# sd196821/QuadSim

Hardware: AMD Instinct MI355X
Metric: env-steps/sec at N parallel envs (1/2/4/8 GPU); per-step state L2 err vs NumPy ref (higher is better)
Workload: dtype f32

## Files before the change

quadsim_amd/csrc/kernel_diag.hpp:

```cpp
#pragma once

#ifdef QS_STAMP
#define QS_STAMP_DECL unsigned long long stamp_[8] = {0, 0, 0, 0, 0, 0, 0, 0}; (void)stamp_
#if QS_STAMP + 0 >= 2
#define QS_STAMP_AT(slot)                                                                                       \
    do {                                                                                                        \
         \
         \
         \
         \
        if ((slot) == 1) stamp_[0] = __builtin_amdgcn_s_memrealtime();                                          \
        else if ((slot) == (role == 0 ? 7 : 6)) {                                                               \
            if (lane == 0 && A.stamps && (tile & 63) == 0) {                    \
                const unsigned long long now_ = __builtin_amdgcn_s_memrealtime();                               \
                const unsigned long long ix_ = ((k0 % 64ull) * (unsigned long long)(A.stamp_tiles) + (unsigned long long)tile) * 16ull + 8 * role; \
                if (ix_ + 8 <= A.stamp_cap) { A.stamps[ix_] = stamp_[0]; A.stamps[ix_ + (slot)] = now_; }       \
            }                                                                                                   \
        }                                                                                                       \
    } while (0)
#else
#define QS_STAMP_AT(slot) (stamp_[slot] = __builtin_amdgcn_s_memrealtime())
#endif
#if QS_STAMP + 0 >= 2
#define QS_STAMP_FLUSH() ((void)0)
#else
#define QS_STAMP_FLUSH()                                                                                        \
    do {                                                                                                        \
        if (lane == 0 && A.stamps) {                                                                            \
            const unsigned long long ix_ = ((k0 % 64ull) * (unsigned long long)(A.stamp_tiles) + (unsigned long long)tile) * 16ull + 8 * role; \
            if (ix_ + 8 <= A.stamp_cap) for (int j_ = 0; j_ < 8; ++j_) A.stamps[ix_ + j_] = stamp_[j_];          \
        }                                                                                                       \
    } while (0)
#endif
#define QS_PHASE_DECL unsigned long long ph_[8] = {0, 0, 0, 0, 0, 0, 0, 0}, ph_t_ = __builtin_amdgcn_s_memrealtime(); \
    const unsigned long long ph_c0_ = __builtin_amdgcn_s_memtime(), ph_r0_ = ph_t_
#define QS_PHASE(slot) do { const unsigned long long n_ = __builtin_amdgcn_s_memrealtime(); ph_[slot] += n_ - ph_t_; ph_t_ = n_; } while (0)
#define QS_PHASE_FLUSH(role_)                                                                                   \
    do {                                                                                                        \
        ph_[6] = __builtin_amdgcn_s_memtime() - ph_c0_;                                   \
        ph_[7] = __builtin_amdgcn_s_memrealtime() - ph_r0_;       \
        if (lane == 0 && A.stamps) {                                                                            \
            const unsigned long long ix_ = (unsigned long long)tile * 16ull + 8 * (role_);                      \
            if (ix_ + 8 <= A.stamp_cap) for (int j_ = 0; j_ < 8; ++j_) A.stamps[ix_ + j_] = ph_[j_];             \
        }                                                                                                       \
    } while (0)
#else
#define QS_STAMP_DECL ((void)0)
#define QS_STAMP_AT(slot) ((void)0)
#define QS_STAMP_FLUSH() ((void)0)
#define QS_PHASE_DECL ((void)0)
#define QS_PHASE(slot) ((void)0)
#define QS_PHASE_FLUSH(role_) ((void)0)
#endif

#if defined(QS_PLAIN_STORES)
#define QS_ST(p, v) (*(p) = (v))
#define QS_SO(p, v) QS_ST(p, v)
#else
#define QS_ST(p, v) __builtin_nontemporal_store((v), (p))
#define QS_SO(p, v) QS_ST(p, v)
#endif
```

quadsim_amd/csrc/private_queue.hpp:

```cpp
#pragma once

struct QsChainLane {
    hsa_queue_t *queue = nullptr;
    char *kernargs = nullptr;
    std::vector<uint64_t> slot_qidx;
    uint64_t issued = 0;
    int64_t tile0 = 0, tile_end = 0;
    hsa_signal_t done{};
    void *rev_ptr = nullptr;
    hsa_signal_t rev{};
    int64_t rev_value = 0;
    char *res_kernarg = nullptr;
    hsa_signal_t res_done{};
    bool res_launched = false;
    uint64_t res_prog = 0;
};

struct QsKernel {
    uint64_t object = 0;
    uint32_t kernarg_size = 0, group_size = 0, private_size = 0;
    unsigned block = 0;
};

struct QsChain {
// ... 375 lines not shown
        memset((char *)p + 4, 0, 60);
        p->signal = wait_sig;
        p->value = wait_value;
        p->mask = -1;
        p->cond = HSA_SIGNAL_CONDITION_GTE;
        p->completion_signal = completion;
        word0 = (uint16_t)((HSA_PACKET_TYPE_VENDOR_SPECIFIC << HSA_PACKET_HEADER_TYPE) | fences) |
                ((uint32_t)HSA_AMD_PACKET_TYPE_BARRIER_VALUE << 16);
    } else {
        hsa_kernel_dispatch_packet_t *p = (hsa_kernel_dispatch_packet_t *)slot;
        const bool res = kind == PKT_RESIDENT;
        p->workgroup_size_x = (uint16_t)(res ? c->res_kernel.block : c->block); p->workgroup_size_y = 1; p->workgroup_size_z = 1;
        p->reserved0 = 0;
        p->grid_size_x = grid; p->grid_size_y = 1; p->grid_size_z = 1;
        p->private_segment_size = res ? c->res_kernel.private_size : c->private_size;
        p->group_segment_size = res ? c->res_kernel.group_size : c->group_size;
        p->kernel_object = res ? c->res_kernel.object : c->kernel_object;
        p->kernarg_address = (void *)kernarg;
        p->reserved2 = 0;
        p->completion_signal = completion;
        word0 = (uint16_t)((HSA_PACKET_TYPE_KERNEL_DISPATCH << HSA_PACKET_HEADER_TYPE) | fences) |
                ((uint32_t)(1 << HSA_KERNEL_DISPATCH_PACKET_SETUP_DIMENSIONS) << 16);
    }
    __atomic_store_n((uint32_t *)slot, word0, __ATOMIC_RELEASE);
    hsa_signal_store_screlease(L.queue->doorbell_signal, (hsa_signal_value_t)idx);
    return idx;
}


double res_now()
{
    timespec ts;
    clock_gettime(CLOCK_MONOTONIC, &ts);
    return (double)ts.tv_sec + 1e-9 * (double)ts.tv_nsec;
}

int res_resolve_kernel(QsEnv *e)
{
    QsChain *c = e->chain;
    if (!c->v_split) { c->res_fits = false; return QS_OK; }
    if (c->res_kernel.object && c->v_integ == c->rv_integ && c->v_params == c->rv_params && c->v_rmode == c->rv_rmode && c->v_prep == c->rv_prep)
        return QS_OK;
    char sym[200];
    snprintf(sym, sizeof sym, "_ZN12_GLOBAL__N_114k_env_residentILi%dELb%dELi%dELi%dEEEvNS_8StepArgsENS_7ResArgsE.kd", c->v_integ,
             c->v_params, c->v_rmode, c->v_prep);
    hsa_executable_symbol_t ks;
    QsKernel k;
    HSA_TRY(hsa_executable_get_symbol_by_name(c->exe, sym, &c->gpu, &ks));
    HSA_TRY(hsa_executable_symbol_get_info(ks, HSA_EXECUTABLE_SYMBOL_INFO_KERNEL_OBJECT, &k.object));
    HSA_TRY(hsa_executable_symbol_get_info(ks, HSA_EXECUTABLE_SYMBOL_INFO_KERNEL_KERNARG_SEGMENT_SIZE, &k.kernarg_size));
    HSA_TRY(hsa_executable_symbol_get_info(ks, HSA_EXECUTABLE_SYMBOL_INFO_KERNEL_GROUP_SEGMENT_SIZE, &k.group_size));
    HSA_TRY(hsa_executable_symbol_get_info(ks, HSA_EXECUTABLE_SYMBOL_INFO_KERNEL_PRIVATE_SEGMENT_SIZE, &k.private_size));
    if (k.kernarg_size > kResKernargBytes) return fail(QS_ERR_HIP, "queue mode: kernel argument block of %s is %u B", sym, k.kernarg_size);
    const int waves = split_waves(c->v_rmode, c->v_prep);
    k.block = (unsigned)(waves * kTile);
    c->res_kernel = k;
    c->rv_integ = c->v_integ; c->rv_params = c->v_params; c->rv_rmode = c->v_rmode; c->rv_prep = c->v_prep;
    c->res_fits = k.private_size == 0 && e->tiles * waves <= c->res_wave_cap;
    return QS_OK;
}

bool res_running(const QsChainLane &L) { return L.res_launched && hsa_signal_load_relaxed(L.res_done) != 0; }

int res_launch(QsEnv *e, QsChainLane &L, uint64_t seq0, uint64_t stop_seq)
{
    QsChain *c = e->chain;
    const size_t q = (size_t)(&L - c->lanes.data());
    StepArgs A = make_args(e);
    A.tile0 = L.tile0; A.tile_end = L.tile_end;
    A.T = 1;
    ResArgs R{};
    R.ring = c->ring;
    R.rseq = c->d_rseq;
    R.wcnt = c->d_rcnt + q * 32;
    R.fin = R.wcnt + kResWinSlots;
    R.h_prog = c->d_hres + q * 8;
    R.h_fin = R.h_prog + 1;
    R.seq0 = seq0;
    R.base = c->res_seq0;
    R.stop_seq = stop_seq;
    R.slots_mask = c->ring_slots - 1;
    R.idle_ticks = c->res_idle_ticks;
    R.lane_tiles = (unsigned)(L.tile_end - L.tile0);
    const size_t roff = (sizeof(StepArgs) + alignof(ResArgs) - 1) / alignof(ResArgs) * alignof(ResArgs);
    memcpy(L.res_kernarg, &A, sizeof A);
    memcpy(L.res_kernarg + roff, &R, sizeof R);
    __builtin_ia32_sfence();
    (void)*(volatile uint32_t *)(L.res_kernarg + roff + sizeof R - sizeof(uint32_t));
    hsa_signal_store_relaxed(L.res_done, 1);
    chain_write_packet(c, L, PKT_RESIDENT, L.res_kernarg, (unsigned)((L.tile_end - L.tile0) * c->res_kernel.block),
                       HSA_FENCE_SCOPE_SYSTEM, HSA_FENCE_SCOPE_SYSTEM, L.res_done);
    L.res_launched = true;
    ++c->res_dispatches;
    return QS_OK;
}

void res_refresh(QsChain *c)
{
    uint64_t m = UINT64_MAX;
    for (size_t q = 0; q < c->lanes.size(); ++q) {
        QsChainLane &L = c->lanes[q];
        L.res_prog = std::max<uint64_t>(L.res_prog, c->h_res[q * 8]);
        m = std::min<uint64_t>(m, L.res_prog);
    }
    c->res_retired = std::max<uint64_t>(c->res_retired, m);
}

int res_write(QsEnv *e, uint64_t s, int cmd, const StepArgs *A)
{
    QsChain *c = e->chain;
    if (c->res_retired + c->ring_slots <= s) {
        const double t_end = res_now() + kResTimeoutS;
        for (;;) {
            res_refresh(c);
            if (c->res_retired + c->ring_slots > s) break;
            for (QsChainLane &L : c->lanes)
                if (L.res_launched && !res_running(L)) { int r = res_launch(e, L, 0, UINT64_MAX); if (r) return r; }
            if (res_now() > t_end)
                return fail(QS_ERR_HIP, "queue mode: the resident step kernel consumed no descriptor for %.0f s (descriptor %llu, all "
                            "consumed below %llu, first lane's progress %llu, %llu dispatches)", kResTimeoutS, (unsigned long long)s,
                            (unsigned long long)c->res_retired, (unsigned long long)c->h_res[0], (unsigned long long)c->res_dispatches);
            __builtin_ia32_pause();
        }
    }
    const unsigned long long p[7] = {
        A ? (unsigned long long)A->actions : 0, A ? (unsigned long long)A->obs : 0, A ? (unsigned long long)A->reward : 0,
        A ? (unsigned long long)A->done : 0, A ? (unsigned long long)A->flags : 0, A ? (unsigned long long)A->term_obs : 0,
        A ? (unsigned long long)A->term_state : 0};
    for (int i = 0; i < 7; ++i)
        if (p[i] & ~kResPtrMask) return fail(QS_ERR_INVALID, "queue mode: a buffer address above 2^48");
    const unsigned long long tag = (unsigned long long)(s & 0xffff) << 48;
    volatile unsigned long long *w = c->ring + (s & (c->ring_slots - 1)) * kResWords;
    for (int i = 0; i < 7; ++i) w[i] = p[i] | tag;
    w[7] = ((unsigned long long)cmd << 32) | (unsigned long long)(uint32_t)(s >> 16) | tag;
    __builtin_ia32_sfence();
    return QS_OK;
}

int res_finish(QsEnv *e)
{
    QsChain *c = e->chain;
    if (!c->res_open) return QS_OK;
    const uint64_t s = c->res_issued;
    int r = res_write(e, s, 1, nullptr);
    if (r) return r;
    c->res_issued = s + 1;
    const double t_end = res_now() + kResTimeoutS;
    for (;;) {
        bool all = true;
        for (size_t q = 0; q < c->lanes.size(); ++q) {
            QsChainLane &L = c->lanes[q];
            if (res_running(L)) { all = false; continue; }
            if (hsa_signal_load_scacquire(L.res_done) == 0 && c->h_res[q * 8 + 1] >= s + 1) continue;
            r = res_launch(e, L, 0, s + 1);
            if (r) return r;
            all = false;
        }
        if (all) break;
        if (res_now() > t_end)
            return fail(QS_ERR_HIP, "queue mode: the resident step kernel did not end within %.0f s of its EXIT descriptor", kResTimeoutS);
        __builtin_ia32_pause();
    }
    c->res_retired = s + 1;
    c->res_open = false;
    return QS_OK;
}
// ... 160 lines not shown
```

quadsim_amd/csrc/quadsim_hip.hip:

```cpp
#include <hip/hip_runtime.h>
#include <hsa/hsa.h>
#include <hsa/hsa_ext_amd.h>
#include <hsa/amd_hsa_signal.h>

#include <elf.h>
#include <fcntl.h>
#include <sys/mman.h>
#include <sys/stat.h>
#include <unistd.h>

#include <cstdarg>
#include <cstdio>
#include <cstdlib>
#include <cstring>
#include <dlfcn.h>
#include <algorithm>
#include <atomic>
#include <condition_variable>
#include <mutex>
#include <new>
#include <thread>
#include <vector>

#ifdef QS_DEBUG
#include <cassert>
#define QS_ASSERT(c) assert(c)
#else
#define QS_ASSERT(c) ((void)0)
#endif

#include "../../include/quadsim.h"
#include "host_util.hpp"
#include "quadsim_device.hpp"
#include "rollout_ops.hpp"
#include "mlp.hpp"

using namespace qs;

#include "kernel_diag.hpp"
#include "step_kernels.hpp"
#include "layer1_kernels.hpp"
#include "policy_kernels.hpp"
#include "runner_kernels.hpp"
#include "expert_rollout.hpp"
#include "shooting.hpp"

#ifdef QS_STAMP
static unsigned long long *g_host_stamps = nullptr;
static unsigned long long g_host_stamp_cap = 0;
#endif

struct QsEnv {
    QsConfig cfg;
    int64_t n = 0, tiles = 0;
    float *st = nullptr, *par = nullptr;
    bool per_env_params = false;
    hipStream_t stream = nullptr;
    bool own_stream = false;
    unsigned long long *d_ctr = nullptr;
    hipEvent_t ev0 = nullptr, ev1 = nullptr;
    float nominal_obs[12] = {0};
    float *gae_ws = nullptr;
    size_t gae_ws_floats = 0;
    float *init = nullptr;
    int obs_dim = 12;
    HostStage stage;
    std::vector<struct QsGroup *> groups;
    hipEvent_t fork_ev = nullptr;
    bool main_dirty = true;
    bool groups_dirty = false;
    bool runner_env_major = false;
    struct QsChain *chain = nullptr;
};

namespace {

StepArgs make_args(const QsEnv *e)
{
    StepArgs A;
    memset(&A, 0, sizeof A);
    A.st = e->st;
    A.par = e->par;
    A.n = e->n;
    A.tile0 = 0; A.tile_end = e->tiles;
    A.io_env0 = 0; A.io_n = e->n;
    A.T = 1;
    A.step_idx = 0;
    A.ctr = e->d_ctr;
    A.gid0 = e->cfg.env_id_offset;
    A.C.kind = e->cfg.kind == QS_KIND_DOCKING_V2 ? 1 : 0;
    A.C.dt = e->cfg.dt;
    A.C.rmax = e->cfg.kind == QS_KIND_DOCKING_V2 ? 10.0f : 3.0f;
    A.C.vdes_x = e->cfg.kind == QS_KIND_DOCKING_V2 ? 0.2f : 0.0f;
    A.init = e->init;
    A.rc.seed = e->cfg.seed;
    for (int i = 0; i < 4; ++i) A.rc.rr[i] = e->cfg.init_range[i];
    A.rc.rr[4] = e->cfg.mass_scale[0]; A.rc.rr[5] = e->cfg.mass_scale[1];
    A.rc.rr[6] = e->cfg.inertia_scale[0]; A.rc.rr[7] = e->cfg.inertia_scale[1];
    A.rc.par_nom[0] = e->cfg.mass;
    for (int i = 0; i < 3; ++i) A.rc.par_nom[1 + i] = e->cfg.inertia[i];
    A.par_nom = Par{e->cfg.mass, e->cfg.inertia[0], e->cfg.inertia[1], e->cfg.inertia[2]};
    A.auto_reset = e->cfg.auto_reset;
    A.randomise = e->cfg.randomise;

    for (int i = 0; i < 12; ++i) A.nominal_obs[i] = e->nominal_obs[i];
#ifdef QS_STAMP
    A.stamps = g_host_stamps; A.stamp_cap = g_host_stamp_cap; A.stamp_tiles = (unsigned long long)e->tiles;
#endif
    return A;
}

UserIO user_io(QsEnv *e) { return UserIO(e->cfg.io_space == QS_IO_HOST ? &e->stage : nullptr, e->stream); }

std::atomic<int> &prep_forced()
{
    static std::atomic<int> f{getenv("QS_RESET_PREP") ? atoi(getenv("QS_RESET_PREP")) : -1};
    return f;
}

int prep_for(int rmode, int64_t tiles)
{
    const int forced = prep_forced().load(std::memory_order_relaxed);
    if (rmode != 1 && rmode != 2) return 0;
    if (forced == 0 || forced == 2) return forced;
    return tiles <= kPrepMaxTiles ? 2 : 0;
}

enum StepFamily { kFamSerial = 0, kFamSplit = 1, kFamResident = 2, kFamChainSplit = 3, kFamChainSerial = 4, kFamHover = 5 };
struct StepVariant {
    int family, integ, params, rmode, prep;
};

// ... 60 lines not shown
    template __global__ void k_env_resident<I, true, 1, 2>(StepArgs, ResArgs);                                          \
    template __global__ void k_env_resident<I, true, 2, 0>(StepArgs, ResArgs);                                          \
    template __global__ void k_env_resident<I, true, 2, 2>(StepArgs, ResArgs);                                          \
    template __global__ void k_env_resident<I, false, 3, 0>(StepArgs, ResArgs);                                         \
    template __global__ void k_env_resident<I, true, 3, 0>(StepArgs, ResArgs);
QS_RES_KERNELS(0)
QS_RES_KERNELS(1)
#undef QS_RES_KERNELS

int launch_env_on(QsEnv *e, const StepArgs &A, hipStream_t s)
{
    const StepVariant v = step_variant(e, A.tile_end - A.tile0);
    if (v.family == kFamHover) {
        const unsigned grid = (unsigned)((A.tile_end - A.tile0 + kBlock / kTile - 1) / (kBlock / kTile));
        with_integ_params(v, [&]<int INTEG, bool PARAMS>() { hipLaunchKernelGGL((k_hover<INTEG, PARAMS>), dim3(grid), dim3(kBlock), 0, s, A); });
    } else with_combo(v, [&]<int INTEG, bool PARAMS, int RMODE>() { launch_one<INTEG, PARAMS, RMODE>(s, A, v); });
    HIP_TRY(hipGetLastError());
    return QS_OK;
}

int launch_env(QsEnv *e, StepArgs &A) { return launch_env_on(e, A, e->stream); }

}

#include "env_groups.hpp"

#include "private_queue.hpp"

namespace {

int main_stream_entry(QsEnv *e)
{
    if (e->groups_dirty) { int rc = groups_join(e); if (rc) return rc; }
    e->main_dirty = true;
    if (e->chain) {
        int rc = chain_drain(e);
        e->chain->hip_dirty = true;
        e->chain->res_dbg_packets = false;
        if (rc) return rc;
    }
    return QS_OK;
}

int fill_params(QsEnv *e)
{
    Par P{e->cfg.mass, e->cfg.inertia[0], e->cfg.inertia[1], e->cfg.inertia[2]};
    hipLaunchKernelGGL(k_fill_par, dim3(grid_tiles(e->n)), dim3(kBlock), 0, e->stream, e->par, e->n, P);
    HIP_TRY(hipGetLastError());
    return QS_OK;
}

int do_reset(QsEnv *e, const uint8_t *d_mask, float *d_obs, int init_all)
{
    StepArgs A = make_args(e);
    A.obs = d_obs;
    if (init_all) A.randomise = 0;
    if (e->cfg.kind == QS_KIND_HOVERING_V0)
        hipLaunchKernelGGL(k_hover_reset, dim3(grid_tiles(e->n)), dim3(kBlock), 0, e->stream, A, d_mask);
    else
        hipLaunchKernelGGL(k_reset, dim3(grid_tiles(e->n)), dim3(kBlock), 0, e->stream, A, d_mask, init_all);
    HIP_TRY(hipGetLastError());
    return QS_OK;
}

#define CHECK_ENV_RAW(e)                                               \
    if (!(e)) return fail(QS_ERR_INVALID, "%s: null handle", __func__); \
    DeviceGuard guard_((e)->cfg.device);                               \
    if (!guard_.ok) return fail(QS_ERR_HIP, "%s: hipSetDevice(%d) failed", __func__, (e)->cfg.device)
#define CHECK_ENV(e)                                                   \
    CHECK_ENV_RAW(e);                                                  \
    if (!(e)->groups.empty() || (e)->chain) { int rcj_ = main_stream_entry(e); if (rcj_) return rcj_; }

}

extern "C" {

int qs_version(void) { return QS_VERSION; }

#ifdef QS_STAMP
int qs_debug_set_stamps(void *dev_ptr, uint64_t capacity_words)
{
    g_host_stamps = (unsigned long long *)dev_ptr;
    g_host_stamp_cap = capacity_words;
    return QS_OK;
}
#endif
const char *qs_last_error(void) { return g_err; }

int qs_debug_step_kernargs(QsEnv *e, const float *actions, float *obs, float *reward, uint8_t *done, uint8_t *flags,
                           float *terminal_obs, void *out, uint64_t cap, uint64_t *size, int32_t *split, int64_t *tiles,
                           int64_t tile0, int64_t tile_end)
{
    if (!e || !out || !size) return fail(QS_ERR_INVALID, "qs_debug_step_kernargs: null argument");
    StepArgs A = make_args(e);
    if (tile_end > tile0) { A.tile0 = tile0; A.tile_end = tile_end; }
    A.actions = actions; A.obs = obs; A.reward = reward; A.done = done; A.flags = flags; A.term_obs = terminal_obs;
    if (cap < sizeof A) return fail(QS_ERR_INVALID, "qs_debug_step_kernargs: buffer too small (%zu needed)", sizeof A);
    memcpy(out, &A, sizeof A);
    *size = sizeof A;
    if (split) *split = split_for(e) ? 1 : 0;
    if (tiles) *tiles = e->tiles;
    return QS_OK;
}

int qs_config_default(QsConfig *cfg)
{
    if (!cfg) return fail(QS_ERR_INVALID, "qs_config_default: null cfg");
    memset(cfg, 0, sizeof *cfg);
    cfg->struct_size = (int32_t)sizeof(QsConfig);
    cfg->kind = QS_KIND_DOCKING_V0;
    cfg->num_envs = 1;
    cfg->device = 0;
    cfg->integrator = QS_INTEG_FROZEN;
    cfg->dt = 0.02f;
    cfg->auto_reset = 0;
    cfg->randomise = QS_RANDOMISE_NONE;
    cfg->io_space = QS_IO_DEVICE;
    cfg->seed = 0;
    cfg->env_id_offset = 0;
    cfg->mass_scale[0] = cfg->mass_scale[1] = 1.0f;
    cfg->inertia_scale[0] = cfg->inertia_scale[1] = 1.0f;
    cfg->mass = 0.18f;
    cfg->inertia[0] = 0.00025f; cfg->inertia[1] = 0.000232f; cfg->inertia[2] = 0.0003738f;
    cfg->stream = nullptr;
    cfg->external_stream = 0;
    return QS_OK;
}

int qs_create(const QsConfig *cfg, QsEnv **out)
{
    if (!cfg || !out) return fail(QS_ERR_INVALID, "qs_create: null argument");
    *out = nullptr;
    if (cfg->struct_size != (int32_t)sizeof(QsConfig))
        return fail(QS_ERR_INVALID, "qs_create: QsConfig size mismatch (got %d, want %zu)", cfg->struct_size, sizeof(QsConfig));
    if (cfg->num_envs < 1) return fail(QS_ERR_INVALID, "qs_create: num_envs must be >= 1");
    if (cfg->num_envs > ((int64_t)1 << 31)) return fail(QS_ERR_INVALID, "qs_create: num_envs too large");
    if (cfg->kind < QS_KIND_DOCKING_V0 || cfg->kind > QS_KIND_HOVERING_V0) return fail(QS_ERR_INVALID, "qs_create: unknown env kind %d", cfg->kind);
    if ((cfg->kind == QS_KIND_DOCKING_V1 || cfg->kind == QS_KIND_HOVERING_V0) && cfg->randomise == QS_RANDOMISE_INIT)
        return fail(QS_ERR_INVALID, "qs_create: docking-v1 / hovering-v0 reset to their stored initial state; randomise must be 0");
    if (cfg->kind == QS_KIND_HOVERING_V0 && cfg->randomise != 0) return fail(QS_ERR_INVALID, "qs_create: hovering-v0 has no randomised resets");
    if (cfg->integrator != QS_INTEG_FROZEN && cfg->integrator != QS_INTEG_RK4) return fail(QS_ERR_INVALID, "qs_create: unknown integrator %d", cfg->integrator);
    if (cfg->randomise < 0 || cfg->randomise > 2) return fail(QS_ERR_INVALID, "qs_create: randomise must be 0..2");
    if (cfg->io_space != QS_IO_DEVICE && cfg->io_space != QS_IO_HOST) return fail(QS_ERR_INVALID, "qs_create: bad io_space");
    if (cfg->randomise && !(cfg->init_range[2] >= 0.0f && cfg->init_range[2] <= 1.5707964f))
        return fail(QS_ERR_INVALID, "qs_create: init_range[2] (euler half-range) must be within [0, pi/2]");
    if (!(cfg->dt > 0.0f) || !(cfg->mass > 0.0f) || !(cfg->inertia[0] > 0.0f) || !(cfg->inertia[1] > 0.0f) || !(cfg->inertia[2] > 0.0f))
        return fail(QS_ERR_INVALID, "qs_create: dt, mass and inertia must be positive");
    int ndev = 0;
    if (hipGetDeviceCount(&ndev) != hipSuccess || ndev <= 0)
        return fail(QS_ERR_NO_DEVICE, "qs_create: no HIP device visible (this library has no CPU fallback)");
    if (cfg->device < 0 || cfg->device >= ndev) return fail(QS_ERR_INVALID, "qs_create: device %d out of range (%d visible)", cfg->device, ndev);
    DeviceGuard guard(cfg->device);
    if (!guard.ok) return fail(QS_ERR_HIP, "qs_create: hipSetDevice(%d) failed", cfg->device);

    QsEnv *e = new (std::nothrow) QsEnv();
    if (!e) return fail(QS_ERR_NOMEM, "qs_create: out of host memory");
    e->cfg = *cfg;
    e->n = cfg->num_envs;
    e->tiles = tiles_of(e->n);
    e->per_env_params = cfg->randomise >= QS_RANDOMISE_PARAMS;
    e->obs_dim = cfg->kind == QS_KIND_HOVERING_V0 ? 13 : 12;
    auto body = [&]() -> int {
        if (cfg->external_stream) e->stream = (hipStream_t)cfg->stream;
        else { HIP_TRY(hipStreamCreateWithFlags(&e->stream, hipStreamNonBlocking)); e->own_stream = true; }
        HIP_TRY(hipEventCreate(&e->ev0));
        HIP_TRY(hipEventCreate(&e->ev1));
// ... 1133 lines not shown
```

quadsim_amd/csrc/step_kernels.hpp:

```cpp
#pragma once

namespace {

#ifndef QS_BLOCK
#define QS_BLOCK 256
#endif
constexpr int kBlock = QS_BLOCK;
#ifndef QS_PREP_MAX_TILES
#define QS_PREP_MAX_TILES 1365
#endif
constexpr int64_t kPrepMaxTiles = QS_PREP_MAX_TILES;
#ifndef QS_SPLIT_MAX_ENVS
#define QS_SPLIT_MAX_ENVS 131072
#endif
constexpr int64_t kSplitMaxEnvs = QS_SPLIT_MAX_ENVS;

struct StepArgs {
    float *st;
    float *par;
    const float *actions;
    float *obs;
    float *reward;
    uint8_t *done;
    uint8_t *flags;
// ... 319 lines not shown
template <bool PARAMS, int RMODE, int PREP>
__device__ __forceinline__ void chaser_reset(const SplitLds<RMODE, PREP> &L, const StepArgs &A, int64_t env, bool active, int lane, int64_t t,
                                             float sc[13], float uc[4], float &ls, float &tt, Par &P, float obs[12])
{
    float ic[13], it[13];
    if (RMODE == 0) {
        nominal_init(ic, it);
#pragma unroll
        for (int i = 0; i < 12; ++i) obs[i] = A.nominal_obs[i];
    } else if (RMODE == 3) {
        const float *src = A.init + (active ? env : 0) * 26;
#pragma unroll
        for (int i = 0; i < 13; ++i) { ic[i] = src[i]; it[i] = src[13 + i]; }
        rel_obs<false>(ic, it, obs);
    } else {
        if constexpr (split_prep(RMODE, PREP)) {
#pragma unroll
            for (int i = 0; i < 13; ++i) ic[i] = L.rst[i][lane];
#pragma unroll
            for (int i = 0; i < 12; ++i) obs[i] = L.rst[13 + i][lane];
            if (PARAMS && RMODE == 2) P = L.reset_par(lane);
        } else {
            const uint4 w0 = L.phx[t & 1][0][lane], w1 = RMODE == 2 ? L.phx[t & 1][1][lane] : make_uint4(0, 0, 0, 0);
            Par Pn;
            random_init_apply<RMODE == 2>(A.rc, w0, w1, ic, it, Pn);
            if (PARAMS && RMODE == 2) P = Pn;
            rel_obs<true>(ic, it, obs);
        }
    }
#pragma unroll
    for (int i = 0; i < 13; ++i) sc[i] = ic[i];
#pragma unroll
    for (int i = 0; i < 4; ++i) uc[i] = 0.0f;
    ls = 0.0f;
    tt = 0.0f;
}

__device__ __forceinline__ void target_load(const float *b, float st[13], float ut[4], float qd[4])
{
#pragma unroll
    for (int i = 0; i < 13; ++i) st[i] = b[(F_ST + i) * kTile];
#pragma unroll
    for (int i = 0; i < 4; ++i) ut[i] = b[(F_UT + i) * kTile];
#pragma unroll
    for (int i = 0; i < 4; ++i) qd[i] = b[(F_QD + i) * kTile];
}

__device__ __forceinline__ void target_store(float *bw, const float st[13], const float ut[4], const float qd[4])
{
#pragma unroll
    for (int i = 0; i < 13; ++i) QS_ST(&bw[(F_ST + i) * kTile], st[i]);
#pragma unroll
    for (int i = 0; i < 4; ++i) QS_ST(&bw[(F_UT + i) * kTile], ut[i]);
#pragma unroll
    for (int i = 0; i < 4; ++i) QS_ST(&bw[(F_QD + i) * kTile], qd[i]);
}

template <int RMODE, int PREP>
__device__ __forceinline__ void target_publish(SplitLds<RMODE, PREP> &L, const StepArgs &A, int64_t env, int lane, uint64_t k, int64_t t,
                                               const float st[13], bool lim_t, uint4 &w0, uint4 &w1)
{
#pragma unroll
    for (int i = 0; i < 13; ++i) L.tgt[i][lane] = st[i];
    L.limt[lane] = lim_t ? 1 : 0;
    w0 = make_uint4(0, 0, 0, 0);
    w1 = w0;
    if constexpr (split_draw(RMODE, PREP)) {
        random_init_words<RMODE == 2>(A.rc, STREAM_AUTORESET, A.gid0 + (uint64_t)env, k + 1, w0, w1);
        L.phx[t & 1][0][lane] = w0;
        if (RMODE == 2) L.phx[t & 1][1][lane] = w1;
    }
}

__device__ __forceinline__ void target_command(const EnvConst &C, float qd[4], const float pre[13], float m, float ut[4])
{
    const float pdes[3] = {10.0f, -50.0f, 5.0f};
    const float vdes[3] = {C.vdes_x, 0.0f, 0.0f};
    const float dv[3] = {0.0f, 0.0f, 0.0f};
    float u_t[4];
    target_control(C.kind, pdes, vdes, qd, 0.0f, pre, dv, m, u_t);
    u_limit(u_t, m * kG, ut);
}

template <bool PARAMS, int RMODE, int PREP>
__device__ __forceinline__ void target_reset(const SplitLds<RMODE, PREP> &L, const StepArgs &A, int64_t env, bool active, int lane,
                                             const uint4 &w0, const uint4 &w1, float st[13], float ut[4], Par &P)
{
    float ic[13], it[13];
    if (RMODE == 3) {
        const float *src = A.init + (active ? env : 0) * 26;
#pragma unroll
        for (int i = 0; i < 13; ++i) it[i] = src[13 + i];
    } else {
        nominal_init(ic, it);
        if (PARAMS && RMODE == 2) {
            if constexpr (split_prep(RMODE, PREP)) {
                P = L.reset_par(lane);
            } else {
                random_init_apply<true>(A.rc, w0, w1, ic, it, P);
                nominal_init(ic, it);
            }
        }
    }
#pragma unroll
    for (int i = 0; i < 13; ++i) st[i] = it[i];
#pragma unroll
    for (int i = 0; i < 4; ++i) ut[i] = 0.0f;
}

template <bool PARAMS, int RMODE, int PREP>
__device__ __forceinline__ void prep_publish(SplitLds<RMODE, PREP> &L, const RandCfg &rc, int lane, const uint4 &w0, const uint4 &w1)
{
    float ic[13], it_[13], robs[12];
    Par Pn;
    random_init_apply<RMODE == 2>(rc, w0, w1, ic, it_, Pn);
    rel_obs<true>(ic, it_, robs);
#pragma unroll
    for (int i = 0; i < 13; ++i) L.rst[i][lane] = ic[i];
#pragma unroll
    for (int i = 0; i < 12; ++i) L.rst[13 + i][lane] = robs[i];
    if (PARAMS && RMODE == 2) {
        L.rst[25][lane] = Pn.m; L.rst[26][lane] = Pn.Ixx; L.rst[27][lane] = Pn.Iyy; L.rst[28][lane] = Pn.Izz;
    }
}

constexpr int kResWords = 8;
constexpr unsigned long long kResPtrMask = (1ull << 48) - 1;
enum { RES_STEP = 0, RES_EXIT = 1, RES_IDLE = 2, RES_SKIP = 3 };
constexpr int kResWin = 32;
constexpr int kResWinSlots = 16;

struct ResArgs {
    const unsigned long long *ring;
    unsigned long long *rseq;
    unsigned *wcnt;
    unsigned *fin;
    unsigned long long *h_prog;
    unsigned long long *h_fin;
    unsigned long long seq0;
    unsigned long long base;
    unsigned long long stop_seq;
    unsigned long long slots_mask;
    unsigned long long idle_ticks;
    unsigned lane_tiles;
};

struct ResDesc {
    const float *actions;
    float *obs, *reward;
    uint8_t *done, *flags;
    float *term_obs, *term_state;
};

__device__ __forceinline__ unsigned long long res_request(const ResArgs &R, unsigned long long s, int lane)
{
    return __hip_atomic_load(R.ring + (s & R.slots_mask) * kResWords + (lane & 7), __ATOMIC_RELAXED, __HIP_MEMORY_SCOPE_SYSTEM);
}

__device__ __forceinline__ bool res_fresh(unsigned long long w, unsigned long long s, int lane)
{
    bool ok = (w >> 48) == (s & 0xffffull);
    if ((lane & 7) == 7) ok = ok && (unsigned)w == (unsigned)(s >> 16);
    return __all(ok);
}

__device__ __forceinline__ unsigned long long res_word(unsigned long long w, int i)
{
    const unsigned lo = (unsigned)__builtin_amdgcn_readlane((int)(unsigned)w, i);
    const unsigned hi = (unsigned)__builtin_amdgcn_readlane((int)(unsigned)(w >> 32), i);
    return (((unsigned long long)hi << 32) | lo) & kResPtrMask;
}

__device__ __forceinline__ int res_resolve(const ResArgs &R, unsigned long long s, int lane, unsigned long long w, ResDesc &D)
{
    if (!res_fresh(w, s, lane)) {
        const unsigned long long t0 = __builtin_amdgcn_s_memrealtime();
        for (;;) {
            __builtin_amdgcn_s_sleep(4);
            w = res_request(R, s, lane);
            if (res_fresh(w, s, lane)) break;
            if (__builtin_amdgcn_s_memrealtime() - t0 > R.idle_ticks) return RES_IDLE;
        }
    }
    D.actions = (const float *)res_word(w, 0);
    D.obs = (float *)res_word(w, 1);
    D.reward = (float *)res_word(w, 2);
    D.done = (uint8_t *)res_word(w, 3);
    D.flags = (uint8_t *)res_word(w, 4);
    D.term_obs = (float *)res_word(w, 5);
    D.term_state = (float *)res_word(w, 6);
    return ((res_word(w, 7) >> 32) & 0xff) == 0 ? RES_STEP : RES_EXIT;
}

__device__ __forceinline__ float4 res_action(const float *actions, int64_t io, int64_t io_n)
{
    typedef unsigned u4 __attribute__((ext_vector_type(4)));
    const __amdgpu_buffer_rsrc_t r = __builtin_amdgcn_make_buffer_rsrc((void *)actions, (short)0, (int)(io_n * 16), 0x00020000);
    const u4 v = __builtin_amdgcn_raw_buffer_load_b128(r, (int)(io * 16), 0, 17);
    return make_float4(__uint_as_float(v.x), __uint_as_float(v.y), __uint_as_float(v.z), __uint_as_float(v.w));
}

__device__ __forceinline__ unsigned res_report(const ResArgs &R, unsigned long long s, int64_t tile, int lane)
{
    const unsigned long long x = s - R.base + (unsigned long long)(tile % kResWin) + 1;
    if (x % kResWin != 0) return ~0u;
    unsigned old = 0;
    if (lane == 0) old = __hip_atomic_fetch_add(R.wcnt + (x / kResWin) % kResWinSlots, 1u, __ATOMIC_RELAXED, __HIP_MEMORY_SCOPE_AGENT);
    return old;
}

__device__ __forceinline__ void res_report_done(const ResArgs &R, unsigned old, unsigned long long s, int64_t tile, int lane)
{
    if (old == ~0u || lane != 0 || (old + 1) % R.lane_tiles != 0) return;
    const unsigned long long x = s - R.base + (unsigned long long)(tile % kResWin) + 1;
    __hip_atomic_store(R.h_prog, R.base + x - kResWin + 1, __ATOMIC_RELAXED, __HIP_MEMORY_SCOPE_SYSTEM);
}

template <int INTEG, bool PARAMS, int RMODE, int PREP>
__global__ __launch_bounds__(3 * kTile) void k_env_resident(StepArgs A, ResArgs R)
{
    __shared__ SplitLds<RMODE, PREP> L;
    __shared__ int s_cmd[2];
    __shared__ unsigned long long s_tsp[2];
    const int lane = threadIdx.x & (kTile - 1);
    const int role = threadIdx.x >> 6;
    const int64_t tile = launch_tile(A, blockIdx.x);
    const int64_t env = tile * kTile + lane;
    bool active = env < A.n;
    const int64_t io = env - A.io_env0;
    QS_ASSERT(tile < A.tile_end && (!active || (io >= 0 && io < A.io_n)));
    const uint64_t k0 = step_counter_begin_vmem(A, tile);
    unsigned long long seq = 0;
    int cmd = RES_STEP;
    ResDesc D{};
    {
        if (role == 0) {
            seq = R.seq0 ? R.seq0 : R.rseq[tile];
            seq = ((unsigned long long)__builtin_amdgcn_readfirstlane((int)(unsigned)(seq >> 32)) << 32) |
                  (unsigned)__builtin_amdgcn_readfirstlane((int)(unsigned)seq);
            cmd = seq >= R.stop_seq ? RES_SKIP : res_resolve(R, seq, lane, res_request(R, seq, lane), D);
            if (cmd == RES_STEP) res_report_done(R, res_report(R, seq, tile, lane), seq, tile, lane);
            if (lane == 0) { s_cmd[0] = cmd; s_tsp[0] = (unsigned long long)D.term_state; }
        }
        __syncthreads();
        cmd = s_cmd[0];
    }
    QS_STAMP_DECL;
    QS_STAMP_AT(0);
    const float *b = A.st + tile * (int64_t)(kRecWords * kTile) + lane;
    float *bw = A.st + tile * (int64_t)(kRecWords * kTile) + lane;
    Par P = A.par_nom;
    if (PARAMS) P = load_par(A.par, tile, lane);
    if (role == 0) {
        __builtin_amdgcn_s_setprio(3);
        float sc[13], uc[4], ls, tt;
        chaser_load(b, sc, uc, ls, tt);
        float4 av_next = make_float4(0.0f, 0.0f, 0.0f, 0.0f);
        if (cmd == RES_STEP && active) av_next = res_action(D.actions, io, A.io_n);
#if defined(QS_STAMP) && QS_STAMP + 0 < 2
        asm volatile("s_waitcnt vmcnt(1)" ::: "memory");
#endif
        QS_STAMP_AT(1);
        int64_t t = 0;
#pragma clang loop unroll(disable)
        for (; cmd == RES_STEP; ++t) {
            const int64_t o = io;
            const unsigned long long wn = res_request(R, seq + t + 1, lane);
            tt += 1.0f;
            const bool lim_c = drone_advance<INTEG>(sc, uc, P, A.C.dt);
            float a[4];
            ResDesc Dn{};
            unsigned rep = ~0u;
            const float4 av = av_next;
            const int cmdn = res_resolve(R, seq + t + 1, lane, wn, Dn);
            if (cmdn == RES_STEP) {
                if (active) av_next = res_action(Dn.actions, io, A.io_n);
                rep = res_report(R, seq + t + 1, tile, lane);
            }
            if (lane == 0) { s_cmd[(t + 1) & 1] = cmdn; s_tsp[(t + 1) & 1] = (unsigned long long)Dn.term_state; }
            a[0] = av.x; a[1] = av.y; a[2] = av.z; a[3] = av.w;
            float u_c[4];
            chaser_command(a, P.m, u_c);
            u_limit(u_c, P.m * kG, uc);
            QS_STAMP_AT(2);
            __syncthreads();
            QS_STAMP_AT(3);
            float obs[12], reward;
            unsigned flags;
            bool done;
            const bool rs = chaser_score(L, lane, sc, a, tt, ls, A.C, A.auto_reset, lim_c, obs, reward, flags, done);
            QS_STAMP_AT(4);
            __syncthreads();
            QS_STAMP_AT(5);
            if (rs) {
                if (D.term_obs && active) store_obs(D.term_obs, io, obs);
                store_term_half(D.term_state, active, io, 0, sc);
                chaser_reset<PARAMS>(L, A, env, active, lane, t, sc, uc, ls, tt, P, obs);
            }
            QS_STAMP_AT(6);
            if (active) {
                store_obs(D.obs, o, obs);
                QS_SO(&D.reward[o], reward);
                QS_SO(&D.done[o], (uint8_t)(done ? 1 : 0));
                if (D.flags) QS_SO(&D.flags[o], (uint8_t)flags);
            }
            res_report_done(R, rep, seq + t + 1, tile, lane);
            D = Dn;
            cmd = cmdn;
        }
        if (t > 0) {
            if (active) {
                chaser_store(bw, sc, uc, ls, tt);
                if (PARAMS && RMODE == 2) store_par(A.par, tile, lane, P);
            }
        }
        {
            if (cmd != RES_SKIP && lane == 0) {
                if (t > 0) A.ctr[tile] = k0 + (uint64_t)t;
                R.rseq[tile] = seq + (unsigned long long)t + (cmd == RES_EXIT ? 1 : 0);
                if (cmd == RES_EXIT) {
                    const unsigned old = __hip_atomic_fetch_add(R.fin, 1u, __ATOMIC_RELAXED, __HIP_MEMORY_SCOPE_AGENT);
                    if (old + 1 == R.lane_tiles)
                        __hip_atomic_store(R.h_fin, seq + (unsigned long long)t + 1, __ATOMIC_RELAXED, __HIP_MEMORY_SCOPE_SYSTEM);
                }
            }
        }
#if defined(QS_STAMP) && QS_STAMP + 0 < 2
        asm volatile("s_waitcnt vmcnt(0)" ::: "memory");
#endif
        QS_STAMP_AT(7);
        QS_STAMP_FLUSH();
    } else if (role == 1) {
        float st[13], ut[4], qd[4];
        target_load(b, st, ut, qd);
#if defined(QS_STAMP) && QS_STAMP + 0 < 2
        asm volatile("s_waitcnt vmcnt(0)" ::: "memory");
#endif
        QS_STAMP_AT(1);
        int64_t t = 0;
#pragma clang loop unroll(disable)
        for (; cmd == RES_STEP; ++t) {
            float pre[13];
#pragma unroll
            for (int i = 0; i < 13; ++i) pre[i] = st[i];
            const bool lim_t = drone_advance<INTEG>(st, ut, P, A.C.dt);
            uint4 w0, w1;
            target_publish(L, A, env, lane, k0 + (uint64_t)t, t, st, lim_t, w0, w1);
            QS_STAMP_AT(2);
            __syncthreads();
            QS_STAMP_AT(3);
            float *const term_state = (float *)s_tsp[t & 1];
            target_command(A.C, qd, pre, P.m, ut);
            QS_STAMP_AT(4);
            __syncthreads();
            QS_STAMP_AT(5);
            if (L.done[lane]) {
                store_term_half(term_state, active, io, 1, st);
                target_reset<PARAMS>(L, A, env, active, lane, w0, w1, st, ut, P);
            }
            cmd = s_cmd[(t + 1) & 1];
        }
        if (active && t > 0) target_store(bw, st, ut, qd);
        QS_STAMP_AT(6);
        QS_STAMP_FLUSH();
    } else if constexpr (split_prep(RMODE, PREP)) {
        int64_t t = 0;
#pragma clang loop unroll(disable)
        for (; cmd == RES_STEP; ++t) {
            uint4 w0, w1 = make_uint4(0, 0, 0, 0);
            random_init_words<RMODE == 2>(A.rc, STREAM_AUTORESET, A.gid0 + (uint64_t)env, k0 + (uint64_t)t + 1, w0, w1);
            __syncthreads();
            prep_publish<PARAMS>(L, A.rc, lane, w0, w1);
            __syncthreads();
            cmd = s_cmd[(t + 1) & 1];
        }
    }
}

template <int INTEG, bool PARAMS, int RMODE, int PREP>
__global__ __launch_bounds__(3 * kTile) void k_env_split(StepArgs A)
{
    __shared__ SplitLds<RMODE, PREP> L;
    const int lane = threadIdx.x & (kTile - 1);
    const int role = threadIdx.x >> 6;
    const int64_t tile = launch_tile(A, blockIdx.x);
    const int64_t env = tile * kTile + lane;
    bool active = env < A.n;
    const int64_t io = env - A.io_env0;
    QS_ASSERT(tile < A.tile_end && (!active || (io >= 0 && io < A.io_n)));
    const unsigned owner_xcc = chain_owner_request(A, tile);
    const uint64_t k0 = step_counter_begin_vmem(A, tile);
    QS_STAMP_DECL;
    QS_STAMP_AT(0);
    const float *b = A.st + tile * (int64_t)(kRecWords * kTile) + lane;
    float *bw = A.st + tile * (int64_t)(kRecWords * kTile) + lane;
    Par P = A.par_nom;
    if (PARAMS) P = load_par(A.par, tile, lane);
    if (role == 0) {
        if (A.T > 1) __builtin_amdgcn_s_setprio(3);
        float sc[13], uc[4], ls, tt;
        chaser_load(b, sc, uc, ls, tt);
        float4 av_next = make_float4(0.0f, 0.0f, 0.0f, 0.0f);
        if (A.actions && active) av_next = reinterpret_cast<const float4 *>(A.actions)[io];
#if defined(QS_STAMP) && QS_STAMP + 0 < 2
        asm volatile("s_waitcnt vmcnt(1)" ::: "memory");
#endif
        QS_STAMP_AT(1);
#pragma clang loop unroll(disable)
        for (int64_t t = 0; t < A.T; ++t) {
            const uint64_t k = k0 + (uint64_t)t;
            const int64_t o = t * A.io_n + io;
            tt += 1.0f;
            const bool lim_c = drone_advance<INTEG>(sc, uc, P, A.C.dt);
            if (A.owner && chain_owner_mismatch(A, tile, lane, owner_xcc)) active = false;
            float a[4];
            if (A.actions) {
                const float4 av = av_next;
                if (t + 1 < A.T && active) av_next = reinterpret_cast<const float4 *>(A.actions)[o + A.io_n];
                a[0] = av.x; a[1] = av.y; a[2] = av.z; a[3] = av.w;
            } else {
                random_action(A.rc.seed, A.gid0 + (uint64_t)env, k, a);
            }
            float u_c[4];
            chaser_command(a, P.m, u_c);
            u_limit(u_c, P.m * kG, uc);
            QS_STAMP_AT(2);
            __syncthreads();
            QS_STAMP_AT(3);
            if (A.T == 1) __builtin_amdgcn_s_setprio(3);
            float obs[12], reward;
            unsigned flags;
            bool done;
            const bool rs = chaser_score(L, lane, sc, a, tt, ls, A.C, A.auto_reset, lim_c, obs, reward, flags, done);
            QS_STAMP_AT(4);
            __syncthreads();
            QS_STAMP_AT(5);
            if (rs) {
                if (A.term_obs && active) store_obs(A.term_obs, io, obs);
                store_term_half(A.term_state, active, io, 0, sc);
                chaser_reset<PARAMS>(L, A, env, active, lane, t, sc, uc, ls, tt, P, obs);
            }
            QS_STAMP_AT(6);
            if (active) {
                if (A.slab) {
                    float2 *row = reinterpret_cast<float2 *>(A.slab + o * 14);
#pragma unroll
                    for (int i = 0; i < 6; ++i) row[i] = make_float2(obs[2 * i], obs[2 * i + 1]);
                    row[6] = make_float2(reward, done ? 1.0f : 0.0f);
                } else {
                    store_obs(A.obs, o, obs);
                    QS_SO(&A.reward[o], reward);
                    QS_SO(&A.done[o], (uint8_t)(done ? 1 : 0));
                }
                if (A.flags) QS_SO(&A.flags[o], (uint8_t)flags);
            }
        }
// ... 266 lines not shown
```

Baseline: 26.95 billion.

## Prefetch resident ring descriptors two steps ahead and set waves-per-EU hint

The resident kernel's chaser loop now issues the ring-descriptor request for step t+2 while resolving step t+1, so the load latency has a full step to hide before the spin-poll check. It also adds an amdgpu_waves_per_eu attribute that depends on the integrator, which changes the register budget given to the compiler. Debug-only recording macros and a record buffer setter are added behind QS_STAMP. Looking further ahead adds an extra live register and a request that may read a slot before it is filled, which relies on the fresh-check and poll logic to stay correct.

Result: slower. 26.66 billion (-1.1%).

```diff
diff --git a/quadsim_amd/csrc/kernel_diag.hpp b/quadsim_amd/csrc/kernel_diag.hpp
--- a/quadsim_amd/csrc/kernel_diag.hpp
+++ b/quadsim_amd/csrc/kernel_diag.hpp
@@ -32,6 +32,27 @@
         }                                                                                                       \
     } while (0)
 #endif
+#if QS_STAMP + 0 < 2
+constexpr unsigned long long kResRecSteps = 64;
+#define QS_RES_REC_DECL unsigned long long rec_top_ = 0, rec_res_ = 0; bool rec_polled_ = false; (void)rec_top_; (void)rec_res_; (void)rec_polled_
+#define QS_RES_REC_TOP() (rec_top_ = __builtin_amdgcn_s_memrealtime())
+#define QS_RES_REC_POLLED , &rec_polled_
+#define QS_RES_REC_RESOLVED() (rec_res_ = __builtin_amdgcn_s_memrealtime())
+#define QS_RES_STAMP_AT(slot) QS_STAMP_AT(slot)
+#define QS_RES_REC(step)                                                                                        \
+    do {                                                                                                        \
+        const unsigned long long x_ = (unsigned long long)(step) - R.rec_k0;                                    \
+        if (R.rec && lane == 0 && (tile & 63) == 0 && x_ < kResRecSteps) {                                      \
+            const unsigned long long ix_ = ((((unsigned long long)tile >> 6) * kResRecSteps + x_) * 3 + (unsigned long long)role) * 8; \
+            if (ix_ + 8 <= R.rec_cap) {                                                                         \
+                unsigned long long *r_ = R.rec + ix_;                                                           \
+                r_[0] = rec_top_; r_[1] = rec_res_;                                                             \
+                for (int j_ = 2; j_ < 7; ++j_) r_[j_] = stamp_[j_];                                             \
+                r_[7] = __builtin_amdgcn_s_memrealtime() | (rec_polled_ ? 1ull << 63 : 0ull);                    \
+            }                                                                                                   \
+        }                                                                                                       \
+    } while (0)
+#endif
 #define QS_PHASE_DECL unsigned long long ph_[8] = {0, 0, 0, 0, 0, 0, 0, 0}, ph_t_ = __builtin_amdgcn_s_memrealtime(); \
     const unsigned long long ph_c0_ = __builtin_amdgcn_s_memtime(), ph_r0_ = ph_t_
 #define QS_PHASE(slot) do { const unsigned long long n_ = __builtin_amdgcn_s_memrealtime(); ph_[slot] += n_ - ph_t_; ph_t_ = n_; } while (0)
@@ -52,6 +73,14 @@
 #define QS_PHASE(slot) ((void)0)
 #define QS_PHASE_FLUSH(role_) ((void)0)
 #endif
+#ifndef QS_RES_REC
+#define QS_RES_REC_DECL ((void)0)
+#define QS_RES_REC_TOP() ((void)0)
+#define QS_RES_REC_POLLED
+#define QS_RES_REC_RESOLVED() ((void)0)
+#define QS_RES_STAMP_AT(slot) ((void)0)
+#define QS_RES_REC(step) ((void)0)
+#endif
 
 #if defined(QS_PLAIN_STORES)
 #define QS_ST(p, v) (*(p) = (v))
diff --git a/quadsim_amd/csrc/private_queue.hpp b/quadsim_amd/csrc/private_queue.hpp
--- a/quadsim_amd/csrc/private_queue.hpp
+++ b/quadsim_amd/csrc/private_queue.hpp
@@ -481,6 +481,9 @@
     R.slots_mask = c->ring_slots - 1;
     R.idle_ticks = c->res_idle_ticks;
     R.lane_tiles = (unsigned)(L.tile_end - L.tile0);
+#ifdef QS_STAMP
+    R.rec = g_res_rec; R.rec_cap = g_res_rec_cap; R.rec_k0 = g_res_rec_k0;
+#endif
     const size_t roff = (sizeof(StepArgs) + alignof(ResArgs) - 1) / alignof(ResArgs) * alignof(ResArgs);
     memcpy(L.res_kernarg, &A, sizeof A);
     memcpy(L.res_kernarg + roff, &R, sizeof R);
diff --git a/quadsim_amd/csrc/quadsim_hip.hip b/quadsim_amd/csrc/quadsim_hip.hip
--- a/quadsim_amd/csrc/quadsim_hip.hip
+++ b/quadsim_amd/csrc/quadsim_hip.hip
@@ -48,6 +48,8 @@
 #ifdef QS_STAMP
 static unsigned long long *g_host_stamps = nullptr;
 static unsigned long long g_host_stamp_cap = 0;
+static unsigned long long *g_res_rec = nullptr;
+static unsigned long long g_res_rec_cap = 0, g_res_rec_k0 = 0;
 #endif
 
 struct QsEnv {
@@ -274,6 +276,13 @@
 {
     g_host_stamps = (unsigned long long *)dev_ptr;
     g_host_stamp_cap = capacity_words;
+    return QS_OK;
+}
+int qs_debug_set_resident_record(void *dev_ptr, uint64_t capacity_words, uint64_t first_step)
+{
+    g_res_rec = (unsigned long long *)dev_ptr;
+    g_res_rec_cap = capacity_words;
+    g_res_rec_k0 = first_step;
     return QS_OK;
 }
 #endif
diff --git a/quadsim_amd/csrc/step_kernels.hpp b/quadsim_amd/csrc/step_kernels.hpp
--- a/quadsim_amd/csrc/step_kernels.hpp
+++ b/quadsim_amd/csrc/step_kernels.hpp
@@ -425,6 +425,18 @@
     u_limit(u_t, m * kG, ut);
 }
 
+__device__ __forceinline__ void target_command_done(float ut[4], float qd[4])
+{
+#ifdef QS_PIN_CONTROLLER
+#pragma unroll
+    for (int i = 0; i < 4; ++i) asm volatile("" : "+v"(ut[i]));
+#pragma unroll
+    for (int i = 0; i < 4; ++i) asm volatile("" : "+v"(qd[i]));
+#else
+    (void)ut; (void)qd;
+#endif
+}
+
 template <bool PARAMS, int RMODE, int PREP>
 __device__ __forceinline__ void target_reset(const SplitLds<RMODE, PREP> &L, const StepArgs &A, int64_t env, bool active, int lane,
                                              const uint4 &w0, const uint4 &w1, float st[13], float ut[4], Par &P)
@@ -486,6 +498,10 @@
     unsigned long long slots_mask;
     unsigned long long idle_ticks;
     unsigned lane_tiles;
+#ifdef QS_STAMP
+    unsigned long long *rec;
+    unsigned long long rec_cap, rec_k0;
+#endif
 };
 
 struct ResDesc {
@@ -514,9 +530,12 @@
     return (((unsigned long long)hi << 32) | lo) & kResPtrMask;
 }
 
-__device__ __forceinline__ int res_resolve(const ResArgs &R, unsigned long long s, int lane, unsigned long long w, ResDesc &D)
-{
+__device__ __forceinline__ int res_resolve(const ResArgs &R, unsigned long long s, int lane, unsigned long long w, ResDesc &D,
+                                           bool *polled = nullptr)
+{
+    if (polled) *polled = false;
     if (!res_fresh(w, s, lane)) {
+        if (polled) *polled = true;
         const unsigned long long t0 = __builtin_amdgcn_s_memrealtime();
         for (;;) {
             __builtin_amdgcn_s_sleep(4);
@@ -560,7 +579,8 @@
 }
 
 template <int INTEG, bool PARAMS, int RMODE, int PREP>
-__global__ __launch_bounds__(3 * kTile) void k_env_resident(StepArgs A, ResArgs R)
+__global__ __launch_bounds__(3 * kTile) __attribute__((amdgpu_waves_per_eu(INTEG == 1 ? 4 : 1)))
+void k_env_resident(StepArgs A, ResArgs R)
 {
     __shared__ SplitLds<RMODE, PREP> L;
     __shared__ int s_cmd[2];
@@ -573,7 +593,7 @@
     const int64_t io = env - A.io_env0;
     QS_ASSERT(tile < A.tile_end && (!active || (io >= 0 && io < A.io_n)));
     const uint64_t k0 = step_counter_begin_vmem(A, tile);
-    unsigned long long seq = 0;
+    unsigned long long seq = 0, wn1 = 0;
     int cmd = RES_STEP;
     ResDesc D{};
     {
@@ -581,7 +601,13 @@
             seq = R.seq0 ? R.seq0 : R.rseq[tile];
             seq = ((unsigned long long)__builtin_amdgcn_readfirstlane((int)(unsigned)(seq >> 32)) << 32) |
                   (unsigned)__builtin_amdgcn_readfirstlane((int)(unsigned)seq);
-            cmd = seq >= R.stop_seq ? RES_SKIP : res_resolve(R, seq, lane, res_request(R, seq, lane), D);
+            if (seq < R.stop_seq) {
+                const unsigned long long w0 = res_request(R, seq, lane);
+                wn1 = res_request(R, seq + 1, lane);
+                cmd = res_resolve(R, seq, lane, w0, D);
+            } else {
+                cmd = RES_SKIP;
+            }
             if (cmd == RES_STEP) res_report_done(R, res_report(R, seq, tile, lane), seq, tile, lane);
             if (lane == 0) { s_cmd[0] = cmd; s_tsp[0] = (unsigned long long)D.term_state; }
         }
@@ -589,6 +615,7 @@
         cmd = s_cmd[0];
     }
     QS_STAMP_DECL;
+    QS_RES_REC_DECL;
     QS_STAMP_AT(0);
     const float *b = A.st + tile * (int64_t)(kRecWords * kTile) + lane;
     float *bw = A.st + tile * (int64_t)(kRecWords * kTile) + lane;
@@ -608,14 +635,21 @@
 #pragma clang loop unroll(disable)
         for (; cmd == RES_STEP; ++t) {
             const int64_t o = io;
-            const unsigned long long wn = res_request(R, seq + t + 1, lane);
+#ifdef QS_AB_LOOKAHEAD1
+            wn1 = res_request(R, seq + t + 1, lane);
+            const unsigned long long wn2 = 0;
+#else
+            const unsigned long long wn2 = res_request(R, seq + t + 2, lane);
+#endif
+            QS_RES_REC_TOP();
             tt += 1.0f;
             const bool lim_c = drone_advance<INTEG>(sc, uc, P, A.C.dt);
             float a[4];
             ResDesc Dn{};
             unsigned rep = ~0u;
             const float4 av = av_next;
-            const int cmdn = res_resolve(R, seq + t + 1, lane, wn, Dn);
+            const int cmdn = res_resolve(R, seq + t + 1, lane, wn1, Dn QS_RES_REC_POLLED);
+            QS_RES_REC_RESOLVED();
             if (cmdn == RES_STEP) {
                 if (active) av_next = res_action(Dn.actions, io, A.io_n);
                 rep = res_report(R, seq + t + 1, tile, lane);
@@ -648,8 +682,10 @@
                 if (D.flags) QS_SO(&D.flags[o], (uint8_t)flags);
             }
             res_report_done(R, rep, seq + t + 1, tile, lane);
+            QS_RES_REC(k0 + (uint64_t)t);
             D = Dn;
             cmd = cmdn;
+            wn1 = wn2;
         }
         if (t > 0) {
             if (active) {
@@ -683,6 +719,7 @@
         int64_t t = 0;
 #pragma clang loop unroll(disable)
         for (; cmd == RES_STEP; ++t) {
+            QS_RES_REC_TOP();
             float pre[13];
 #pragma unroll
             for (int i = 0; i < 13; ++i) pre[i] = st[i];
@@ -694,6 +731,7 @@
             QS_STAMP_AT(3);
             float *const term_state = (float *)s_tsp[t & 1];
             target_command(A.C, qd, pre, P.m, ut);
+            target_command_done(ut, qd);
             QS_STAMP_AT(4);
             __syncthreads();
             QS_STAMP_AT(5);
@@ -701,6 +739,7 @@
                 store_term_half(term_state, active, io, 1, st);
                 target_reset<PARAMS>(L, A, env, active, lane, w0, w1, st, ut, P);
             }
+            QS_RES_REC(k0 + (uint64_t)t);
             cmd = s_cmd[(t + 1) & 1];
         }
         if (active && t > 0) target_store(bw, st, ut, qd);
@@ -710,11 +749,17 @@
         int64_t t = 0;
 #pragma clang loop unroll(disable)
         for (; cmd == RES_STEP; ++t) {
+            QS_RES_REC_TOP();
             uint4 w0, w1 = make_uint4(0, 0, 0, 0);
             random_init_words<RMODE == 2>(A.rc, STREAM_AUTORESET, A.gid0 + (uint64_t)env, k0 + (uint64_t)t + 1, w0, w1);
+            QS_RES_STAMP_AT(2);
             __syncthreads();
+            QS_RES_STAMP_AT(3);
             prep_publish<PARAMS>(L, A.rc, lane, w0, w1);
+            QS_RES_STAMP_AT(4);
             __syncthreads();
+            QS_RES_STAMP_AT(5);
+            QS_RES_REC(k0 + (uint64_t)t);
             cmd = s_cmd[(t + 1) & 1];
         }
     }
```
